# ShunyaoWang/quadruped_locomotion

Measured on AMD Instinct MI355X. Metric: control-step QP solves/sec (18-DoF, 4-contact) at 1/2/4/8 MI355X, higher is better.
Workload: dtype f64

## Files before the change

### quadruped_locomotion_amd/csrc/balance_coop.hpp

```cpp
#pragma once

#include "force_qp_coop.hpp"
#include "kernarg_mirror.hpp"
#include "qlamd.h"

namespace qlamd {
namespace coop {

struct CoopPtrs {
  const double *q, *pos, *quat, *linvel, *angvel, *dpos, *dquat, *dlinvel, *dangvel;
  const uint8_t *stance;
  const double *normals;
  const double *wrench;
  const uint8_t *live;
  int support_only;
  int32_t *iterations;
  const uint32_t *prev_working_set;
  uint32_t *working_set;
  uint32_t *warm_retries;
  int record_doubles;
  uint32_t *set_memory;
};

__host__ __device__ constexpr unsigned slot_legs_of(unsigned m) {
  unsigned perm = 0, k = 0;
  for (unsigned l = 0; l < 4; l++)
    if ((m >> l) & 1u) perm |= l << (2 * k++);
  for (unsigned l = 0; l < 4; l++)
    if (!((m >> l) & 1u)) perm |= l << (2 * k++);
  return perm;
}
__host__ __device__ constexpr unsigned long long slot_legs_table(int half) {
  unsigned long long t = 0;
  for (int m = 0; m < 8; m++) t |= (unsigned long long)slot_legs_of(8 * half + m) << (8 * m);
  return t;
}
__device__ __forceinline__ unsigned slot_legs(unsigned m) {
  constexpr unsigned long long lo = slot_legs_table(0), hi = slot_legs_table(1);
  return (unsigned)(((m & 8u) ? hi : lo) >> (8 * (m & 7u))) & 0xFFu;
}
template <int kKinds, class mask_t>
__device__ __forceinline__ mask_t working_set_to_slots(mask_t by_leg, unsigned perm) {
  constexpr mask_t rows = ((mask_t)1 << kKinds) - 1;
  mask_t out = 0;
#pragma unroll
  for (int sl = 0; sl < 4; sl++) out |= ((by_leg >> (kKinds * ((perm >> (2 * sl)) & 3u))) & rows) << (kKinds * sl);
  return out;
}
template <int kKinds, class mask_t>
__device__ __forceinline__ mask_t working_set_to_legs(mask_t by_slot, unsigned perm) {
  constexpr mask_t rows = ((mask_t)1 << kKinds) - 1;
  mask_t out = 0;
#pragma unroll
  for (int sl = 0; sl < 4; sl++) out |= ((by_slot >> (kKinds * sl)) & rows) << (kKinds * ((perm >> (2 * sl)) & 3u));
  return out;
}
__device__ __forceinline__ double from_leg_lane(double v, int aleg) {
  const int addr = (((int)threadIdx.x & 48) | (4 * aleg) | ((int)threadIdx.x & 3)) << 2;
  return __hiloint2double(__builtin_amdgcn_ds_bpermute(addr, __double2hiint(v)),
                          __builtin_amdgcn_ds_bpermute(addr, __double2loint(v)));
}

constexpr int kCoopNrmDoubles = 12 * 64;

template <bool kPerLeg, int kBlock = 64, bool kWarm = false, bool kParkInputs = false, bool kThroughput = false, bool kSmallForm = true,
          bool kTable = false>
__device__ __forceinline__ bool coop_robot(const DeviceParams &P, const CoopPtrs &s, int64_t irobot, bool robot_live_in,
                                           double *lds_tab, double *lds_row, double *lds_nrm,
                                           double *__restrict__ tau_out,
                                           double *__restrict__ grf_out, int32_t *__restrict__ status_out, bool cold = false) {
  bool robot_live = robot_live_in;
  const int lr = threadIdx.x & 15;
  const int leg = lr >> 2, c = lr & 3;
  const bool comp = c < 3;
  const int myidx = 3 * leg + c;
  const double eps = 2.220446049250313e-16;
  const double inf = INFINITY;

  QL_STAMP(0);
  constexpr int kTabLoads = (4 * kTabPerLeg + kBlock - 1) / kBlock;
  double tabv[kTabLoads];
#pragma unroll
  for (int j = 0; j < kTabLoads; j++) {
    const int idx = (int)threadIdx.x + kBlock * j;
    tabv[j] = P.legtab[idx < 4 * kTabPerLeg ? idx : 4 * kTabPerLeg - 1];
  }
  const int64_t i_in = irobot;
  const int64_t kS12 = s.record_doubles ? s.record_doubles : 12, kS4 = s.record_doubles ? s.record_doubles : 4,
                kS3 = s.record_doubles ? s.record_doubles : 3, kSB = 4;
  double quat[4], dquat[4], pos[3], linvel[3], angvel[3], dpos[3], dlinvel[3], dangvel[3];
  {
    const double2 *a2 = reinterpret_cast<const double2 *>(s.quat + kS4 * i_in);
    const double2 *b2 = reinterpret_cast<const double2 *>(s.dquat + kS4 * i_in);
    double2 v = a2[0]; quat[0] = v.x; quat[1] = v.y;
    v = a2[1]; quat[2] = v.x; quat[3] = v.y;
    v = b2[0]; dquat[0] = v.x; dquat[1] = v.y;
    v = b2[1]; dquat[2] = v.x; dquat[3] = v.y;
#pragma unroll
    for (int k = 0; k < 3; k++) {
      pos[k] = s.pos[kS3 * i_in + k]; linvel[k] = s.linvel[kS3 * i_in + k]; angvel[k] = s.angvel[kS3 * i_in + k];
      dpos[k] = s.dpos[kS3 * i_in + k]; dlinvel[k] = s.dlinvel[kS3 * i_in + k]; dangvel[k] = s.dangvel[kS3 * i_in + k];
    }
  }
  const uint32_t sm = *reinterpret_cast<const uint32_t *>(s.stance + kSB * i_in);
  double qj = s.q[kS12 * i_in + (comp ? myidx : 0)];
  const uint8_t alive = s.live ? s.live[i_in] : (uint8_t)1;
  unsigned warm_set = 0u;
  bool build_set = false;
  static_assert(!kTable || kWarm, "the table is a warm start");
  uint4 mem = make_uint4(0u, 0u, 0u, 0u);
  if constexpr (kTable) mem = reinterpret_cast<const uint4 *>(s.set_memory)[i_in];
  else if constexpr (kWarm) warm_set = (s.prev_working_set && !cold) ? s.prev_working_set[i_in] : 0u;
  double wr[6] = {0.0, 0.0, 0.0, 0.0, 0.0, 0.0};
  if (s.wrench) {
#pragma unroll
    for (int k = 0; k < 6; k++) wr[k] = s.wrench[6 * i_in + k];
  }
  double nWl[3] = {0.0, 0.0, 1.0};
  if (kPerLeg) { nWl[0] = s.normals[12 * i_in + 3 * leg]; nWl[1] = s.normals[12 * i_in + 3 * leg + 1]; nWl[2] = s.normals[12 * i_in + 3 * leg + 2]; }
  robot_live = robot_live && alive != 0;
  const unsigned stance = robot_live ? (((sm & 0xFFu) ? 1u : 0u) | ((sm & 0xFF00u) ? 2u : 0u) |
                                        ((sm & 0xFF0000u) ? 4u : 0u) | ((sm & 0xFF000000u) ? 8u : 0u))
                                     : 0u;
  const int nS = __popc(stance);
  if constexpr (kTable) {
    const unsigned slot = QLAMD_SET_MEMORY_SLOT(stance);
    warm_set = slot == 0u ? mem.x : slot == 1u ? mem.y : slot == 2u ? mem.z : mem.w;
  }
  if constexpr (kWarm) {
    const unsigned from = (warm_set >> 20) & 0xFu;
    warm_set = (from != 0u && from != stance) ? 0u : (warm_set & 0xFFFFFu);
    if constexpr (kTable) build_set = from != stance;
    else build_set = s.prev_working_set != nullptr && !cold && from != stance;
  }
  const unsigned perm = slot_legs(stance);
  const int aleg = (int)((perm >> (2 * leg)) & 3u);
  reinterpret_cast<int2 *>(lds_nrm + 64 * 11)[(int)threadIdx.x & 63] = make_int2((int)i_in, (3 * aleg + c) | ((int)perm << 8) | ((int)stance << 16));
  const bool on = leg < nS;
  const unsigned stance_slots = (1u << nS) - 1u;
  const bool permuted = __builtin_amdgcn_ballot_w64(perm != 0xE4u) != 0ull;
  if (permuted) {
    qj = from_leg_lane(qj, aleg);
    if (kPerLeg) { nWl[0] = from_leg_lane(nWl[0], aleg); nWl[1] = from_leg_lane(nWl[1], aleg); nWl[2] = from_leg_lane(nWl[2], aleg); }
  }
#pragma unroll
  for (int j = 0; j < kTabLoads; j++) {
    const int idx = (int)threadIdx.x + kBlock * j;
    if (idx < 4 * kTabPerLeg) lds_tab[idx] = tabv[j];
  }
  __syncthreads();

  QL_STAMP(1); QL_QP_BLOCK_STAMP(4);
  double Rm[9], gB[3], b[6];
  double wr_d[3] = {0.0, 0.0, 0.0}, wr_dw = 1.0, wr_k = 2.0;
  bool wr_slow = false;
  quat_to_matrix(quat, Rm);
  {
    const double gW[3] = {0.0, 0.0, -P.grav};
    irot(Rm, gW, gB);
    RobotIn in;
#pragma unroll
    for (int k = 0; k < 3; k++) {
      in.pos[k] = pos[k]; in.linvel[k] = linvel[k]; in.angvel[k] = angvel[k];
      in.dpos[k] = dpos[k]; in.dlinvel[k] = dlinvel[k]; in.dangvel[k] = dangvel[k];
    }
#pragma unroll
    for (int k = 0; k < 4; k++) { in.quat[k] = quat[k]; in.dquat[k] = dquat[k]; }
    in.has_wrench = false;
    wr_dw = 0.0;
    {
      const double *qd = in.dquat, *qm = in.quat;
      const double aw = qd[0], ax = -qd[1], ay = -qd[2], az = -qd[3];
      wr_dw = aw * qm[0] - ax * qm[1] - ay * qm[2] - az * qm[3];
      wr_d[0] = aw * qm[1] + ax * qm[0] + ay * qm[3] - az * qm[2];
      wr_d[1] = aw * qm[2] - ax * qm[3] + ay * qm[0] + az * qm[1];
      wr_d[2] = aw * qm[3] + ax * qm[2] - ay * qm[1] + az * qm[0];
      const double s2r = 1.0 - wr_dw * wr_dw;
      const double s2 = vmin(vmax(s2r, 0.0), 0.01);
      double p = 34459425.0 / 3530096640.0;
      p = fma(p, s2, 2027025.0 / 175472640.0);
      p = fma(p, s2, 135135.0 / 9676800.0);
      p = fma(p, s2, 10395.0 / 599040.0);
      p = fma(p, s2, 945.0 / 42240.0);
      p = fma(p, s2, 105.0 / 3456.0);
      p = fma(p, s2, 15.0 / 336.0);
      p = fma(p, s2, 3.0 / 40.0);
      p = fma(p, s2, 1.0 / 6.0);
      p = fma(p, s2, 1.0);
      wr_k = 2.0 * p;
      wr_slow = !(s2r < 0.01) || !(wr_dw > 0.0);
    }
    {
      double e_p[3], e_v[3], e_w[3];
#pragma unroll
      for (int k = 0; k < 3; k++) {
        e_p[k] = in.dpos[k] - in.pos[k];
        e_v[k] = in.dlinvel[k] - in.linvel[k];
        e_w[k] = in.dangvel[k] - in.angvel[k];
      }
      const double ff[3] = {in.dlinvel[0], in.dlinvel[1], 0.0};
      const double gfb[3] = {0.0, 0.0, P.kp_t[2] * e_p[2]};
      const double gdb[3] = {0.0, 0.0, P.kd_t[2] * e_v[2]};
// ... 47 lines not shown
    for (int a = 0; a < 3; a++) Rn[a] = Rc[0] * Rs[a] + Rc[1] * Rs[3 + a] + Rc[2] * Rs[6 + a];
    Rc[0] = Rn[0]; Rc[1] = Rn[1]; Rc[2] = Rn[2];
    Hk[k] = m * pc + (Rn[0] * mcom[0] + Rn[1] * mcom[1] + Rn[2] * mcom[2]);
    if (k < 3) { zax[k] = Rn[2]; pj[k] = pc; }
  }
  const double foot = (comp && on) ? pc : 0.0;
  const auto qcross = [&](double a, double bq) -> double {
    const double a1 = dpp<0xC9>(a), a2 = dpp<0xD2>(a);
    const double b1 = dpp<0xC9>(bq), b2 = dpp<0xD2>(bq);
    return a1 * b2 - a2 * b1;
  };
  double Jrow[3], Gq[3];
  {
    const double my_g = pick3(gB, c);
    double Hs = Hk[3];
    double M = tab[kTabMass + 3];
#pragma unroll
    for (int k = 2; k >= 0; k--) {
      Hs += Hk[k];
      M += tab[kTabMass + k];
      const double d = pc - pj[k];
      const double jc = qcross(zax[k], d);
      Jrow[k] = sel(comp, jc, 0.0);
      const double h = Hs - M * pj[k];
      const double zh = qcross(zax[k], h);
      Gq[k] = -quad_sum(sel(comp, my_g * zh, 0.0));
    }
  }

  if (__builtin_amdgcn_ballot_w64(wr_slow) != 0ull) {
    const double s2 = 1.0 - wr_dw * wr_dw;
    double k = 2.0;
    if (s2 >= 1e-12) k = 2.0 * acos(wr_dw) / sqrt(s2);
    const double dk = wr_slow ? k - wr_k : 0.0;
#pragma unroll
    for (int a = 0; a < 3; a++) b[3 + a] -= P.kp_r[a] * dk * wr_d[a];
  }
  if (s.wrench) {
#pragma unroll
    for (int k = 0; k < 6; k++) b[k] = wr[k];
  }
#pragma unroll
  for (int k = 0; k < 3; k++) {
    lds_nrm[64 * (5 + k) + ((int)threadIdx.x & 63)] = Jrow[k];
    lds_nrm[64 * (8 + k) + ((int)threadIdx.x & 63)] = Gq[k];
  }
  asm volatile("" ::: "memory");
  static_assert(!kParkInputs || kBlock == 64, "the parked inputs take the model table's place: one wavefront per workgroup");
  if constexpr (kParkInputs) {
    lds_tab[(int)threadIdx.x & 63] = foot;
#pragma unroll
    for (int k = 0; k < 6; k++) lds_tab[64 + 6 * (((int)threadIdx.x & 63) >> 4) + k] = b[k];
  }

  QL_STAMP(3); QL_QP_BLOCK_STAMP(5);
  double myn = 0.0, myt1 = 0.0, myt2 = 0.0;
  double nb[3], t1[3], t2[3];
  {
    const double ey[3] = {0.0, 1.0, 0.0}, ez[3] = {0.0, 0.0, 1.0};
    double yB[3], nW[3];
    irot(Rm, ey, yB);
    if (kPerLeg) { nW[0] = nWl[0]; nW[1] = nWl[1]; nW[2] = nWl[2]; }
    else rot(Rm, ez, nW);
    irot(Rm, nW, nb);
    cross3(nb, yB, t1);
    double nn = rsqrt_nr(dot3(t1, t1));
    t1[0] *= nn; t1[1] *= nn; t1[2] *= nn;
    cross3(nb, t1, t2);
    nn = rsqrt_nr(dot3(t2, t2));
    t2[0] *= nn; t2[1] *= nn; t2[2] *= nn;
    myn = pick3(nb, c); myt1 = pick3(t1, c); myt2 = pick3(t2, c);
  }
  const double mu = P.mu, f_min = P.f_min;

  QL_STAMP(4);
  QL_STAMP(5);
  double x;
  int qp_iters;
  unsigned long long final_set = 0ull;
  const bool two_legs = __builtin_amdgcn_ballot_w64(nS > 2) == 0ull;
  int status = kStatusOk;
  const auto solve = [&](auto Legs) {
    ForceQp Q;
    if constexpr (kParkInputs) {
      asm volatile("" ::: "memory");
      const double foot_l = lds_tab[(int)threadIdx.x & 63];
      double b_l[6];
#pragma unroll
      for (int k = 0; k < 6; k++) b_l[k] = lds_tab[64 + 6 * (((int)threadIdx.x & 63) >> 4) + k];
      force_qp_objective(P.S, P.w_reg, foot_l, stance_slots, comp && on, b_l, nullptr, 0.0, Q.Gm, Q.g0);
    } else {
      force_qp_objective(P.S, P.w_reg, foot, stance_slots, comp && on, b, nullptr, 0.0, Q.Gm, Q.g0);
    }
#pragma unroll
    for (int k = 0; k < 3; k++) { Q.nb[k] = nb[k]; Q.t1[k] = t1[k]; Q.t2[k] = t2[k]; }
    Q.myn = myn; Q.myt1 = myt1; Q.myt2 = myt2;
    Q.mu = mu; Q.f_min = f_min;
    Q.on = on; Q.comp = comp; Q.nS = nS; Q.refine_passes = P.refine_passes;
    Q.warm = 0ull; Q.stance = stance_slots;
    Q.build_set = build_set;
    if constexpr (kWarm) Q.warm = permuted ? working_set_to_slots<5, unsigned>(warm_set, perm) : warm_set;
    status = force_qp_coop<false, kWarm, decltype(Legs)::value, !kThroughput>(Q, lds_row, lds_nrm, x, qp_iters, &final_set);
  };
  if constexpr (kSmallForm) {
    int small_form = __builtin_amdgcn_readfirstlane(two_legs ? 1 : 0);
    asm volatile("" : "+s"(small_form));
    if (small_form != 0) solve(std::integral_constant<int, 2>{});
    int large_form = __builtin_amdgcn_readfirstlane(1 - small_form);
    asm volatile("" : "+s"(large_form));
    if (large_form != 0) solve(std::integral_constant<int, 4>{});
  } else {
    (void)two_legs;
    solve(std::integral_constant<int, 4>{});
  }
  const int2 parked = reinterpret_cast<const int2 *>(lds_nrm + 64 * 11)[(int)threadIdx.x & 63];
  const int64_t i = parked.x;
  const int aidx = parked.y & 15;
  if constexpr (kWarm) {
    if (permuted) final_set = working_set_to_legs<5, unsigned>((unsigned)final_set, ((unsigned)parked.y >> 8) & 0xFFu);
  }
  if (status == kStatusNotPd) {
    if (lr == 0 && robot_live) {
      status_out[i] = kStatusNotPd;
      if (s.iterations) s.iterations[i] = 0;
      if constexpr (kWarm) { if (s.working_set) s.working_set[i] = 0u; }
      if constexpr (kTable) s.set_memory[4 * i + QLAMD_SET_MEMORY_SLOT((unsigned)parked.y >> 16)] = 0u;
    }
    if (comp && robot_live && !P.keep_on_failure && (on || !s.support_only)) { tau_out[12 * i + aidx] = 0.0; if (grf_out) grf_out[12 * i + aidx] = 0.0; }
    return false;
  }

  QL_STAMP(8);
  {
    const bool live = on && status == kStatusOk;
    const double fx = live ? -x : 0.0;
    double Jr[3], Gr[3];
#pragma unroll
    for (int k = 0; k < 3; k++) {
      Jr[k] = lds_nrm[64 * (5 + k) + ((int)threadIdx.x & 63)];
      Gr[k] = lds_nrm[64 * (8 + k) + ((int)threadIdx.x & 63)];
    }
    const double t0 = quad_sum(sel(comp, Jr[0] * fx, 0.0)) + Gr[0];
    const double t1 = quad_sum(sel(comp, Jr[1] * fx, 0.0)) + Gr[1];
    const double t2 = quad_sum(sel(comp, Jr[2] * fx, 0.0)) + Gr[2];
    double t = sel(c == 0, t0, sel(c == 1, t1, t2));
    t = t > P.tau_max ? P.tau_max : t;
    t = t < -P.tau_max ? -P.tau_max : t;
    if (comp && robot_live && !(P.keep_on_failure && status != kStatusOk) && (on || !s.support_only)) {
      tau_out[12 * i + aidx] = live ? t : 0.0;
      if (grf_out) grf_out[12 * i + aidx] = live ? x : 0.0;
    }
    if (lr == 0 && robot_live) {
      status_out[i] = status;
      if (s.iterations) s.iterations[i] = qp_iters;
      if constexpr (kWarm) {
        const uint32_t word = status == kStatusOk ? ((uint32_t)final_set | (((uint32_t)parked.y >> 16 & 0xFu) << 20)) : 0u;
        if (s.working_set) s.working_set[i] = word;
        if constexpr (kTable)
          s.set_memory[4 * i + QLAMD_SET_MEMORY_SLOT((unsigned)parked.y >> 16)] = (P.warm_fallback == 2 && final_set != 0ull) ? 0u : word;
      }
    }
  }
  QL_STAMP(9);
  QL_STAMP(10);
  const bool rejected = kWarm && robot_live && (status == kStatusWarmRejected || (P.warm_fallback == 2 && status == kStatusOk && final_set != 0ull));
  if constexpr (kWarm) {
    if (rejected && lr == 0 && s.warm_retries) atomicAdd(s.warm_retries, 1u);
  }
  return rejected;
}

template <class Args>
__device__ __forceinline__ const Args *kernel_arguments_again() {
  typedef __attribute__((address_space(4))) const char kernarg_char;
  kernarg_char *kp = (kernarg_char *)__builtin_amdgcn_kernarg_segment_ptr();
  asm volatile("" : "+s"(kp));
  return (const Args *)kp;
}

}
}
```

### quadruped_locomotion_amd/csrc/balance_core.hpp

```cpp
#pragma once

#include <math.h>
#include <stdint.h>

#if defined(__HIPCC__)
#define QL_HD __host__ __device__ __forceinline__
#define QL_UNROLL _Pragma("unroll")
#define QL_NOUNROLL _Pragma("nounroll")
#define QL_HD_CALL __host__ __device__ __attribute__((noinline))
#else
#define QL_HD inline
#define QL_UNROLL
#define QL_NOUNROLL
#define QL_HD_CALL inline
#endif

namespace qlamd {

constexpr int kStatusOk = 0, kStatusInfeasible = 1, kStatusNotPd = 2, kStatusMaxIter = 3, kStatusDependentEquality = 5;
constexpr int kMaxOuter = 200;

struct DeviceParams {
  double kp_t[3], kd_t[3], kff_t[3];
  double kp_r[3], kd_r[3], kff_r[3];
  double S[6];
  double w_reg, mu, f_min, tau_max;
  double grav;
  double Fg_scale;
  double Tg_arm[3];
  double legtab[4 * 88];
  int refine_passes;
  int keep_on_failure;
  int warm_fallback;
};
constexpr int kTabR0 = 0, kTabXyz = 36, kTabMass = 48, kTabMcom = 52, kTabInertia = 64, kTabPerLeg = 88;

struct RobotIn {
  double q[12];
  double pos[3], quat[4], linvel[3], angvel[3];
  double dpos[3], dquat[4], dlinvel[3], dangvel[3];
  unsigned stance;
  bool has_wrench;
  double wrench[6];
};

#if defined(__HIP_DEVICE_COMPILE__)
QL_HD double ql_rcp(double x) {
  double y = __builtin_amdgcn_rcp(x);
  y = y + y * (1.0 - x * y);
  y = y + y * (1.0 - x * y);
  return y;
}
QL_HD double ql_rsqrt(double x) {
  double y = __builtin_amdgcn_rsq(x);
  y = y + y * (0.5 - 0.5 * x * y * y);
  y = y + y * (0.5 - 0.5 * x * y * y);
  return y;
}
#else
QL_HD double ql_rcp(double x) { return 1.0 / x; }
QL_HD double ql_rsqrt(double x) { return 1.0 / sqrt(x); }
#endif


QL_HD void cross3(const double a[3], const double b[3], double c[3]) {
  c[0] = a[1] * b[2] - a[2] * b[1];
  c[1] = a[2] * b[0] - a[0] * b[2];
  c[2] = a[0] * b[1] - a[1] * b[0];
}
QL_HD double dot3(const double a[3], const double b[3]) { return a[0] * b[0] + a[1] * b[1] + a[2] * b[2]; }

QL_HD void sincos_pio4(double x, double &s, double &c) {
  const double z = x * x;
  const double S1 = -1.66666666666666324348e-01, S2 = 8.33333333332248946124e-03,
               S3 = -1.98412698298579493134e-04, S4 = 2.75573137070700676789e-06,
               S5 = -2.50507602534068634195e-08, S6 = 1.58969099521155010221e-10;
  const double C1 = 4.16666666666666019037e-02, C2 = -1.38888888888741095749e-03,
               C3 = 2.48015872894767294178e-05, C4 = -2.75573143513906633035e-07,
               C5 = 2.08757232129817482790e-09, C6 = -1.13596475577881948265e-11;
  const double ps = S1 + z * (S2 + z * (S3 + z * (S4 + z * (S5 + z * S6))));
  s = x + x * z * ps;
  const double pc = z * (C1 + z * (C2 + z * (C3 + z * (C4 + z * (C5 + z * C6)))));
  c = 1.0 - (0.5 * z - z * pc);
}
QL_HD void sincos_reduced(double x, double &s, double &c) {
  const double two_over_pi = 6.36619772367581382433e-01;
  const double pio2_hi = 1.57079632673412561417e+00;
  const double pio2_lo = 6.07710050650619224932e-11;
  const double kf = rint(x * two_over_pi);
  const int k = (int)kf;
  const double r = (x - kf * pio2_hi) - kf * pio2_lo;
  double sr, cr;
  sincos_pio4(r, sr, cr);
  const bool swap = (k & 1) != 0;
  const double s0 = swap ? cr : sr, c0 = swap ? sr : cr;
  s = (k & 2) ? -s0 : s0;
  c = ((k + 1) & 2) ? -c0 : c0;
}

QL_HD void quat_to_matrix(const double q[4], double R[9]) {
  const double w = q[0], x = q[1], y = q[2], z = q[3];
  const double tx = 2.0 * x, ty = 2.0 * y, tz = 2.0 * z;
  const double twx = tx * w, twy = ty * w, twz = tz * w;
  const double txx = tx * x, txy = ty * x, txz = tz * x;
  const double tyy = ty * y, tyz = tz * y, tzz = tz * z;
  R[0] = 1.0 - (tyy + tzz); R[1] = txy - twz;         R[2] = txz + twy;
  R[3] = txy + twz;         R[4] = 1.0 - (txx + tzz); R[5] = tyz - twx;
  R[6] = txz - twy;         R[7] = tyz + twx;         R[8] = 1.0 - (txx + tyy);
}
QL_HD void rot(const double R[9], const double v[3], double o[3]) {
  QL_UNROLL for (int i = 0; i < 3; i++) o[i] = R[i * 3] * v[0] + R[i * 3 + 1] * v[1] + R[i * 3 + 2] * v[2];
}
QL_HD void irot(const double R[9], const double v[3], double o[3]) {
// ... 605 lines not shown
```

### quadruped_locomotion_amd/csrc/force_qp_coop.hpp

```cpp
#pragma once

#include "coop_lanes.hpp"

#if defined(__FAST_MATH__) || (defined(__FINITE_MATH_ONLY__) && __FINITE_MATH_ONLY__)
#error "force_qp_coop.hpp needs IEEE inf / NaN semantics: do not build this translation unit with -ffast-math / -ffinite-math-only"
#endif

#ifndef QL_QP_BLOCK_STAMP
#define QL_QP_BLOCK_STAMP(slot) QL_BLOCK_STAMP(slot)
#endif
namespace qlamd {
namespace coop {

constexpr int kCoopLdsDoubles = 12 * 12;
constexpr int kMaxRefinePasses = 8;
#ifndef QLAMD_REFINE_AGAIN
#define QLAMD_REFINE_AGAIN 1e-3
#endif
constexpr double kRefineAgain = QLAMD_REFINE_AGAIN;
constexpr int kDropSlot = 48, kZeroSlot = 60, kWarmSlot = 61;
constexpr int kForceQpNrmRows = 5, kForceQpNrmRowsTorque = 8;
template <class T>
constexpr T one_v = T(1);
constexpr int kStatusWarmRejected = 6;
struct ForceQp {
  double Gm[12];
  double g0;
  double nb[3], t1[3], t2[3];
  double myn, myt1, myt2;
  double mu, f_min;
  bool on, comp;
  int nS;
  int refine_passes;
  double jrow[3], jcol[3];
  double tq_up, tq_lo;
  unsigned long long warm;
  unsigned stance;
  bool build_set;
};

__device__ __forceinline__ void force_qp_objective(const double S[6], double w_reg, double foot, unsigned stance, bool row_on,
                                                   const double F[6], const double *jrow, double w_tau_jt0, double Gm[12],
                                                   double &g0, double w_tau = 0.0) {
  const int lr = threadIdx.x & 15, leg = lr >> 2, c = lr & 3;
  const int myidx = 3 * leg + c;
  double r[4][3];
  static_for<12>([&](auto J) { constexpr int j = J; r[j / 3][j % 3] = bcv<j>(foot); });
  const double rl[3] = {quad_bc<0>(foot), quad_bc<1>(foot), quad_bc<2>(foot)};
  const double a[3] = {sel(c == 1, -rl[2], sel(c == 2, rl[1], 0.0)), sel(c == 0, rl[2], sel(c == 2, -rl[0], 0.0)),
                       sel(c == 0, -rl[1], sel(c == 1, rl[0], 0.0))};
  const double sa[3] = {S[3] * a[0], S[4] * a[1], S[5] * a[2]};
  const double Sfc = pick3(S, c);
#pragma unroll
  for (int m = 0; m < 4; m++) {
    const bool both = row_on && ((stance >> m) & 1u);
    const double xp = r[m][0], yp = r[m][1], zp = r[m][2];
    const double e0 = sa[1] * zp - sa[2] * yp;
    const double e1 = -sa[0] * zp + sa[2] * xp;
    const double e2 = sa[0] * yp - sa[1] * xp;
    Gm[3 * m + 0] = both ? e0 + (c == 0 ? Sfc : 0.0) : 0.0;
    Gm[3 * m + 1] = both ? e1 + (c == 1 ? Sfc : 0.0) : 0.0;
    Gm[3 * m + 2] = both ? e2 + (c == 2 ? Sfc : 0.0) : 0.0;
  }
  if (jrow) {
    double jj[3];
    static_for<3>([&](auto Bq) {
      constexpr int bq = Bq;
      jj[bq] = jrow[0] * quad_bc<bq>(jrow[0]) + jrow[1] * quad_bc<bq>(jrow[1]) + jrow[2] * quad_bc<bq>(jrow[2]);
    });
#pragma unroll
    for (int m = 0; m < 4; m++) {
      const bool own = row_on && m == leg;
#pragma unroll
      for (int bq = 0; bq < 3; bq++) Gm[3 * m + bq] += own ? w_tau * jj[bq] : 0.0;
    }
  }
#pragma unroll
  for (int j = 0; j < 12; j++)
    if (c < 3 && j == myidx) Gm[j] += row_on ? w_reg : 1.0;
  const double Fc = pick3(F, c);
  const double ST[3] = {S[3] * F[3], S[4] * F[4], S[5] * F[5]};
  const double g0v = -(Sfc * Fc + (a[0] * ST[0] + a[1] * ST[1] + a[2] * ST[2]) + w_tau_jt0);
  g0 = sel(row_on, g0v, 0.0);
}

template <bool kTorque, bool kWarm = false, int kLegs = 4, bool kRounds = true>
__device__ __forceinline__ int force_qp_coop(const ForceQp &Q, double *lds_row, double *lds_nrm, double &x, int &iters_out,
                                             unsigned long long *ws_out = nullptr) {
  using mask_t = std::conditional_t<kTorque, unsigned long long, unsigned>;
  constexpr int kKinds = kTorque ? 11 : 5;
  static_assert(kLegs == 2 || kLegs == 4, "legs in front of the row");
  constexpr int kV = 3 * kLegs;
  const int lr = threadIdx.x & 15, leg = lr >> 2, c = lr & 3;
  const bool comp = Q.comp && leg < kLegs, on = Q.on, row_on = comp && on;
  const int myidx = 3 * leg + c, nS = Q.nS;
  const double eps = 2.220446049250313e-16;
  const double inf = INFINITY;
  const double mu = Q.mu, f_min = Q.f_min, g0 = Q.g0;
  const double myn = Q.myn, myt1 = Q.myt1, myt2 = Q.myt2;
  const double *nb = Q.nb, *t1 = Q.t1, *t2 = Q.t2, *Gm = Q.Gm;
  double H[kV];
  double c1 = 0.0, c2 = 0.0;
  {
#pragma unroll
    for (int j = 0; j < kV; j++) H[j] = Gm[j];
    {
      double diag = 0.0;
#pragma unroll
      for (int j = 0; j < kV; j++) diag = (j == myidx) ? Gm[j] : diag;
      c1 = row_sum(sel(row_on, diag, 0.0));
    }
    bool bad = false;
    double my_pivot = 1.0;
    double d = bcv<0>(H[0]);
    static_for<kV>([&](auto K) {
      constexpr int k = K;
      bad = bad || !(d > 0.0);
      const double p = rcp_nr1(d);
      const bool piv = comp && (myidx == k);
      my_pivot = piv ? d : my_pivot;
      const double f = piv ? (1.0 - p) : H[k] * p;
      const double nf = -f;
      if constexpr (k < kV - 1) {
        fmac_bc<lane_of(k), true>(H[k + 1], H[k + 1], nf);
        d = bcv<k + 1>(H[k + 1]);
      }
      static_for<kV>([&](auto J) {
        constexpr int j = J;
        if constexpr (j != k && j != k + 1) fmac_bc<lane_of(k), (k == kV - 1 && j == 0)>(H[j], H[j], nf);
      });
      H[k] = piv ? p : nf;
    });
    const double rp = rsqrt_nr(my_pivot);
    c2 = row_sum(sel(row_on, rp, 0.0));
    if (bad && nS > 0) { iters_out = 0; return kStatusNotPd; }
  }

  QL_STAMP(5);
  x = 0.0;
  {
    const double ng0 = -g0;
    double xa[3] = {0.0, 0.0, 0.0};
    static_for<kV>([&](auto J) { constexpr int j = J; fmac_bc<lane_of(j), j == 0>(xa[j % 3], ng0, H[j]); });
    x = (xa[0] + xa[1]) + xa[2];
  }

  QL_STAMP(6); QL_QP_BLOCK_STAMP(6);
  double Ns[kV];
#pragma unroll
  for (int j = 0; j < kV; j++) Ns[j] = 0.0;
  double u = 0.0;
  int idk = 0;
  unsigned used = 0;
  int q = 0, iters = 0, status = kStatusOk;
  mask_t act_mask = 0, excl = 0;
  const double psi_tol = (double)(kKinds * nS) * eps * c1 * c2 * 100.0;
  double rnorm2 = 1.0;
  unsigned long long done_m = 0ull;
  int ip = 0;
  double sp = 0.0, ucand = 0.0, npj = 0.0;
  const double fa = c == 0 ? 1.0 : c == 1 ? -1.0 : 0.0, fb = c == 2 ? 1.0 : c == 3 ? -1.0 : 0.0;
  const double Wf0 = mu * nb[0] + (fa * t1[0] + fb * t2[0]), Wf1 = mu * nb[1] + (fa * t1[1] + fb * t2[1]),
               Wf2 = mu * nb[2] + (fa * t1[2] + fb * t2[2]);
  const mask_t one = 1;
  const mask_t maskf = on ? (one << (kKinds * leg + c + 1)) : 0, maskm = (on && c == 0) ? (one << (kKinds * leg)) : 0;
  const mask_t masku = (kTorque && on && comp) ? (one << (kKinds * leg + 5 + 2 * c)) : 0, maskl = masku << 1;
  constexpr int kTagBits = kTorque ? 2 : 1;
  constexpr unsigned kTagMask = (1u << (4 + kTagBits)) - 1u;
  const unsigned tagf = (unsigned)lr << kTagBits, tagm = tagf | 1u;
  const int row_addr = ((int)threadIdx.x & 48) << 2;
  const unsigned lanebit = 1u << lr;
  {
    const double nrm[5] = {myn, mu * myn + myt1, mu * myn - myt1, mu * myn + myt2, mu * myn - myt2};
#pragma unroll
    for (int k = 0; k < 5; k++) lds_nrm[64 * k + ((int)threadIdx.x & 63)] = nrm[k];
    lds_row[kZeroSlot] = 0.0;
    if constexpr (kTorque) {
#pragma unroll
      for (int k = 0; k < 3; k++) lds_nrm[64 * (5 + k) + ((int)threadIdx.x & 63)] = Q.jrow[k];
    }
  }
  const int nt_slot = comp ? kDropSlot + myidx : kZeroSlot;
  double zb = 0.0;
  double s_up = 0.0, s_lo = 0.0;
  const auto slacks = [&](double xx, double &s_min, double &s_fric) {
    const double x0 = quad_bc<0>(xx), x1 = quad_bc<1>(xx), x2 = quad_bc<2>(xx);
    s_fric = fma(Wf2, x2, fma(Wf1, x1, Wf0 * x0));
    s_min = fma(nb[2], x2, fma(nb[1], x1, fma(nb[0], x0, -f_min)));
    if constexpr (kTorque) {
      const double d = fma(Q.jcol[2], x2, fma(Q.jcol[1], x1, Q.jcol[0] * x0));
      s_up = Q.tq_up + d;
      s_lo = Q.tq_lo - d;
    }
  };
  const auto violation = [&](double s_min, double s_fric) -> double {
    double v = vmin(0.0, s_fric) + sel(c == 0, vmin(0.0, s_min), 0.0);
    if constexpr (kTorque) v += sel(comp, vmin(0.0, s_up) + vmin(0.0, s_lo), 0.0);
    return v;
  };
  const auto umax_dpp = [](unsigned k, auto Ctrl) -> unsigned {
    constexpr int ctrl = decltype(Ctrl)::value;
    const unsigned o = (unsigned)__builtin_amdgcn_mov_dpp((int)k, ctrl, 0xF, 0xF, true);
    return k > o ? k : o;
  };

  const auto latch = [&](bool newly) {
    if (newly) {
      lds_row[lr] = x;
      reinterpret_cast<int2 *>(lds_row + 16)[lr] = make_int2((int)used, idk);
      reinterpret_cast<int2 *>(lds_row + 32)[lr] = make_int2(q | (iters << 8), status);
      lds_row[nt_slot] = 0.0;
      lds_nrm[64 * 1 + ((int)threadIdx.x & 63)] = 0.0;
      zb = 0.0625; npj = 0.0;
    }
  };
  double vec = 0.0, hc = 0.0, nc = 0.0;
  const auto update_and_select = [&](auto Mode, bool resel, bool fresh, bool finished = false) -> bool {
    constexpr int kMode = decltype(Mode)::value;
    constexpr bool kUpd = kMode != 0;
    if constexpr (kMode == 1) {
      iters += (resel && fresh) ? 1 : 0;
      excl = (resel && fresh) ? 0 : excl;
    } else {
// ... 550 lines not shown
```

### quadruped_locomotion_amd/csrc/params_build.hpp

```cpp
#pragma once

#include <math.h>
#include <stdlib.h>
#include <string.h>

#include "balance_core.hpp"
#include "qlamd.h"
#include "qlamd_robot_constants.h"

namespace qlamd {

inline void default_balance_params(qlamd_balance_params *p) {
  const double kp_t[3] = {5000, 5000, 10000}, kd_t[3] = {5000, 4000, 5000}, kff_t[3] = {10, 10, 100};
  const double kp_r[3] = {10000, 10000, 4000}, kd_r[3] = {1000, 1000, 1000}, kff_r[3] = {0.2, 0.2, 1000};
  const double S[6] = {1, 5, 1, 10, 10, 5};
  const double hips[4][3] = {{0.42, 0.075, 0.0}, {0.42, -0.075, 0.0}, {-0.42, -0.075, 0.0}, {-0.42, 0.075, 0.0}};
  memcpy(p->kp_trans, kp_t, sizeof(kp_t)); memcpy(p->kd_trans, kd_t, sizeof(kd_t));
  memcpy(p->kff_trans, kff_t, sizeof(kff_t));
  memcpy(p->kp_rot, kp_r, sizeof(kp_r)); memcpy(p->kd_rot, kd_r, sizeof(kd_r));
  memcpy(p->kff_rot, kff_r, sizeof(kff_r));
  memcpy(p->force_weights, S, sizeof(S));
  p->regularizer = 0.0001; p->friction = 0.6; p->min_normal_force = 10.0;
  p->torque_limit = 300.0;
  p->torso_mass = 27.0;
  for (int i = 0; i < 4; i++) p->leg_mass[i] = 6.0;
  p->gravity = 9.8;
  p->grav_comp_percentage = 1.0;
  p->com_in_base[0] = p->com_in_base[1] = p->com_in_base[2] = 0.0;
  memcpy(p->hip_in_base, hips, sizeof(hips));
}

inline void default_robot_model(qlamd_robot_model *m) {
  memcpy(m->joint_xyz, QLAMD_JOINT_XYZ, sizeof(m->joint_xyz));
  memcpy(m->joint_rpy, QLAMD_JOINT_RPY, sizeof(m->joint_rpy));
  memcpy(m->link_mass, QLAMD_LINK_MASS, sizeof(m->link_mass));
  memcpy(m->link_com, QLAMD_LINK_COM, sizeof(m->link_com));
  memcpy(m->link_inertia, QLAMD_LINK_INERTIA, sizeof(m->link_inertia));
  m->base_mass = QLAMD_BASE_MASS;
  memcpy(m->base_com, QLAMD_BASE_COM, sizeof(m->base_com));
  memcpy(m->base_inertia, QLAMD_BASE_INERTIA, sizeof(m->base_inertia));
}

inline void rpy_to_matrix(const double rpy[3], double R[9]) {
  const double cr = cos(rpy[0]), sr = sin(rpy[0]);
  const double cp = cos(rpy[1]), sp = sin(rpy[1]);
  const double cy = cos(rpy[2]), sy = sin(rpy[2]);
  R[0] = cy * cp; R[1] = cy * sp * sr - sy * cr; R[2] = cy * sp * cr + sy * sr;
  R[3] = sy * cp; R[4] = sy * sp * sr + cy * cr; R[5] = sy * sp * cr - cy * sr;
  R[6] = -sp;     R[7] = cp * sr;                R[8] = cp * cr;
}

inline void build_device_params(const qlamd_balance_params &p, const qlamd_robot_model &m, DeviceParams *d) {
  memset(d, 0, sizeof(*d));
  for (int i = 0; i < 3; i++) {
    d->kp_t[i] = p.kp_trans[i]; d->kd_t[i] = p.kd_trans[i]; d->kff_t[i] = p.kff_trans[i];
    d->kp_r[i] = p.kp_rot[i];   d->kd_r[i] = p.kd_rot[i];   d->kff_r[i] = p.kff_rot[i];
  }
  for (int i = 0; i < 6; i++) d->S[i] = p.force_weights[i];
  d->w_reg = p.regularizer; d->mu = p.friction; d->f_min = p.min_normal_force; d->tau_max = p.torque_limit;
  d->grav = p.gravity;
  d->refine_passes = 1;
  d->keep_on_failure = 0;
  d->warm_fallback = 1;
  double mass = p.torso_mass;
  double arm[3] = {p.torso_mass * p.com_in_base[0], p.torso_mass * p.com_in_base[1], p.torso_mass * p.com_in_base[2]};
  for (int l = 0; l < 4; l++) {
    mass += p.leg_mass[l];
    for (int i = 0; i < 3; i++) arm[i] += p.leg_mass[l] * (p.hip_in_base[l][i] - p.com_in_base[i]);
  }
  d->Fg_scale = p.grav_comp_percentage * mass;
  for (int i = 0; i < 3; i++) d->Tg_arm[i] = p.grav_comp_percentage * arm[i];
  for (int l = 0; l < 4; l++) {
    double *tab = d->legtab + kTabPerLeg * l;
    for (int k = 0; k < 4; k++) {
      rpy_to_matrix(m.joint_rpy[l][k], tab + kTabR0 + 9 * k);
      tab[kTabMass + k] = m.link_mass[l][k];
      for (int i = 0; i < 3; i++) {
        tab[kTabXyz + 3 * k + i] = m.joint_xyz[l][k][i];
        tab[kTabMcom + 3 * k + i] = m.link_mass[l][k] * m.link_com[l][k][i];
      }
      for (int i = 0; i < 6; i++) tab[kTabInertia + 6 * k + i] = m.link_inertia[l][k][i];
    }
  }
}

}
```

### quadruped_locomotion_amd/csrc/balance_coop_body.hpp

```cpp
  double *tab = lds, *rows = lds + 4 * kTabPerLeg, *nrm = rows + 4 * kCoopWaves * coop::kCoopLdsDoubles;
  const DeviceParams &P = *Pp;
  const int row = threadIdx.x >> 4, wave = threadIdx.x >> 6;
  unsigned block = blockIdx.x;
  QL_BLOCK_STAMP(0);
  if constexpr (kPlaced) {
    if (s.shadow_blocks) {
      if (block < (unsigned)s.shadow_blocks) {
        placement_wave(s.prev_iterations, B, s.place_throughput, s.next_order, (lds_u32 *)lds, block, (uint32_t)s.shadow_blocks,
                       (uint32_t)s.shadow_chunk, s.place_throughput ? reinterpret_cast<const uint32_t *>(s.stance) : nullptr, s.place_hist, s.place_sync,
                       s.place_wait);
        return;
      }
      block -= (unsigned)s.shadow_blocks;
      __builtin_amdgcn_s_setprio(3);
    }
  }
  int64_t i = (int64_t)block * (4 * kCoopWaves) + row;
  bool live = i < B;
  if (!live) i = B - 1;
  if constexpr (kPlaced) {
    if constexpr (kMinWaves == 2) {
      if (s.shadow_blocks == 0 && s.next_order && live && (threadIdx.x & 15) == 0) s.next_order[i] = (int32_t)i;
    }
    if (s.order) {
      const int64_t o = s.order[i];
      live = live && o >= 0 && o < B;
      i = live ? o : B - 1;
    }
  }
  const coop::CoopPtrs cp{s.q, s.pos, s.quat, s.linvel, s.angvel, s.dpos, s.dquat, s.dlinvel, s.dangvel, s.stance,
                          s.normals, s.wrench, s.live, s.support_only, kPlaced ? s.iterations : nullptr,
                          kWarm ? s.prev_working_set : nullptr, kWarm ? s.working_set : nullptr, kWarm ? s.warm_retries : nullptr,
                          s.record_doubles, kTable ? s.set_memory : nullptr};
#ifdef QLAMD_STAMPS
#pragma unroll 1
  for (int rep = 0; rep < 2; rep++)
#endif
  {
    const bool rejected = coop::coop_robot<kPerLeg, 64 * kCoopWaves, kWarm, kMinWaves == 3 && !kWarm && kPlaced, kMinWaves == 3, kPlaced, kTable>(
        P, cp, i, live, tab, rows + row * coop::kCoopLdsDoubles, nrm + wave * coop::kCoopNrmDoubles, tau, grf, status);
    QL_BLOCK_STAMP(3);
    if constexpr (kWarm) {
      if (__builtin_expect(P.warm_fallback && __builtin_amdgcn_ballot_w64(rejected) != 0ull, 0)) {
        __syncthreads();
        if constexpr (kTable) balance_table_retry<kPerLeg, kMinWaves>(coop::kernel_arguments_again<BalanceCoopArgs>(), lds, rejected);
        else balance_cold_retry<kPerLeg, kMinWaves>(coop::kernel_arguments_again<BalanceCoopArgs>(), lds, rejected);
      }
    }
  }
```

Baseline: 299.9 million.

## Replace Gauss-Jordan Hessian inverse with closed-form structured inverse for 4-leg force QP

Adds a closed-form inverse of the force-QP Hessian that exploits its structure: diagonal regularizer plus low-rank wrench terms, reduced to a 3x3 Schur complement per row. It is used for the non-torque, 4-leg case and falls back to the cooperative Gauss-Jordan elimination when any lane detects ill-conditioning. The goal is to remove the serial cross-lane elimination cost. In exchange it adds precomputed sqrt and inverse parameters, extra fields in the QP struct, and possible numerical differences compared with the elimination path.

```diff
diff --git a/quadruped_locomotion_amd/csrc/balance_coop.hpp b/quadruped_locomotion_amd/csrc/balance_coop.hpp
--- a/quadruped_locomotion_amd/csrc/balance_coop.hpp
+++ b/quadruped_locomotion_amd/csrc/balance_coop.hpp
@@ -331,15 +331,17 @@
   int status = kStatusOk;
   const auto solve = [&](auto Legs) {
     ForceQp Q;
+    double b_l[6];
     if constexpr (kParkInputs) {
       asm volatile("" ::: "memory");
       const double foot_l = lds_tab[(int)threadIdx.x & 63];
-      double b_l[6];
 #pragma unroll
       for (int k = 0; k < 6; k++) b_l[k] = lds_tab[64 + 6 * (((int)threadIdx.x & 63) >> 4) + k];
-      force_qp_objective(P.S, P.w_reg, foot_l, stance_slots, comp && on, b_l, nullptr, 0.0, Q.Gm, Q.g0);
+      force_qp_objective(P.S, P.w_reg, foot_l, stance_slots, comp && on, b_l, nullptr, 0.0, Q.Gm, Q.g0, 0.0, &Q.foot);
+      Q.F = b_l;
     } else {
-      force_qp_objective(P.S, P.w_reg, foot, stance_slots, comp && on, b, nullptr, 0.0, Q.Gm, Q.g0);
+      force_qp_objective(P.S, P.w_reg, foot, stance_slots, comp && on, b, nullptr, 0.0, Q.Gm, Q.g0, 0.0, &Q.foot);
+      Q.F = b;
     }
 #pragma unroll
     for (int k = 0; k < 3; k++) { Q.nb[k] = nb[k]; Q.t1[k] = t1[k]; Q.t2[k] = t2[k]; }
@@ -348,6 +350,7 @@
     Q.on = on; Q.comp = comp; Q.nS = nS; Q.refine_passes = P.refine_passes;
     Q.warm = 0ull; Q.stance = stance_slots;
     Q.build_set = build_set;
+    Q.inv = StructuredInverseParams{P.S, P.S_sqrt, P.w_reg, P.w_reg_inv, P.w_reg_rsqrt};
     if constexpr (kWarm) Q.warm = permuted ? working_set_to_slots<5, unsigned>(warm_set, perm) : warm_set;
     status = force_qp_coop<false, kWarm, decltype(Legs)::value, !kThroughput>(Q, lds_row, lds_nrm, x, qp_iters, &final_set);
   };
diff --git a/quadruped_locomotion_amd/csrc/balance_core.hpp b/quadruped_locomotion_amd/csrc/balance_core.hpp
--- a/quadruped_locomotion_amd/csrc/balance_core.hpp
+++ b/quadruped_locomotion_amd/csrc/balance_core.hpp
@@ -29,6 +29,8 @@
   double Fg_scale;
   double Tg_arm[3];
   double legtab[4 * 88];
+  double S_sqrt[6];
+  double w_reg_inv, w_reg_rsqrt;
   int refine_passes;
   int keep_on_failure;
   int warm_fallback;
diff --git a/quadruped_locomotion_amd/csrc/force_qp_coop.hpp b/quadruped_locomotion_amd/csrc/force_qp_coop.hpp
--- a/quadruped_locomotion_amd/csrc/force_qp_coop.hpp
+++ b/quadruped_locomotion_amd/csrc/force_qp_coop.hpp
@@ -1,6 +1,7 @@
 #pragma once
 
 #include "coop_lanes.hpp"
+#include "force_qp_inverse.hpp"
 
 #if defined(__FAST_MATH__) || (defined(__FINITE_MATH_ONLY__) && __FINITE_MATH_ONLY__)
 #error "force_qp_coop.hpp needs IEEE inf / NaN semantics: do not build this translation unit with -ffast-math / -ffinite-math-only"
@@ -36,14 +37,19 @@
   double tq_up, tq_lo;
   unsigned long long warm;
   unsigned stance;
+  double foot;
+  const double *F;
+  StructuredInverseParams inv;
   bool build_set;
 };
 
 __device__ __forceinline__ void force_qp_objective(const double S[6], double w_reg, double foot, unsigned stance, bool row_on,
                                                    const double F[6], const double *jrow, double w_tau_jt0, double Gm[12],
-                                                   double &g0, double w_tau = 0.0) {
+                                                   double &g0, double w_tau = 0.0, double *foot_on = nullptr) {
   const int lr = threadIdx.x & 15, leg = lr >> 2, c = lr & 3;
   const int myidx = 3 * leg + c;
+  foot = sel(row_on, foot, 0.0);
+  if (foot_on) *foot_on = foot;
   double r[4][3];
   static_for<12>([&](auto J) { constexpr int j = J; r[j / 3][j % 3] = bcv<j>(foot); });
   const double rl[3] = {quad_bc<0>(foot), quad_bc<1>(foot), quad_bc<2>(foot)};
@@ -101,7 +107,23 @@
   const double *nb = Q.nb, *t1 = Q.t1, *t2 = Q.t2, *Gm = Q.Gm;
   double H[kV];
   double c1 = 0.0, c2 = 0.0;
-  {
+#ifdef QLAMD_NO_STRUCTURED_INVERSE
+  constexpr bool kStructured = false;
+#else
+  constexpr bool kStructured = !kTorque && kLegs == 4;
+#endif
+  bool gauss_jordan = !kStructured;
+  x = 0.0;
+  if constexpr (kStructured) {
+    double r[4][3];
+    static_for<12>([&](auto J) { constexpr int j = J; r[j / 3][j % 3] = bcv<j>(Q.foot); });
+    const double rl[3] = {quad_bc<0>(Q.foot), quad_bc<1>(Q.foot), quad_bc<2>(Q.foot)};
+    bool ill;
+    const bool bad = structured_inverse_row<4>(Q.inv, r, rl, Q.stance, nS, leg, c, comp, row_on, Q.F, H, c1, c2, x, ill);
+    if (bad && nS > 0) { iters_out = 0; return kStatusNotPd; }
+    gauss_jordan = __builtin_amdgcn_ballot_w64(ill && nS > 0) != 0ull;
+  }
+  if (gauss_jordan) {
 #pragma unroll
     for (int j = 0; j < kV; j++) H[j] = Gm[j];
     {
@@ -137,8 +159,7 @@
   }
 
   QL_STAMP(5);
-  x = 0.0;
-  {
+  if (gauss_jordan) {
     const double ng0 = -g0;
     double xa[3] = {0.0, 0.0, 0.0};
     static_for<kV>([&](auto J) { constexpr int j = J; fmac_bc<lane_of(j), j == 0>(xa[j % 3], ng0, H[j]); });
diff --git a/quadruped_locomotion_amd/csrc/force_qp_inverse.hpp b/quadruped_locomotion_amd/csrc/force_qp_inverse.hpp
--- /dev/null
+++ b/quadruped_locomotion_amd/csrc/force_qp_inverse.hpp
@@ -0,0 +1,77 @@
+#pragma once
+
+#include "balance_core.hpp"
+
+namespace qlamd {
+
+struct StructuredInverseParams {
+  const double *S, *S_sqrt;
+  double w, w_inv, w_rsqrt;
+};
+
+QL_HD double si_sel(bool p, double a, double b) { return p ? a : b; }
+template <int kLegs>
+QL_HD bool structured_inverse_row(const StructuredInverseParams &P, const double (*r)[3], const double rl[3], unsigned stance, int n,
+                                  int leg, int c, bool comp, bool row_on, const double F[6], double *H, double &c1, double &c2, double &x0,
+                                  bool &ill) {
+  const double *S = P.S, *s = P.S_sqrt;
+  const double w = P.w, g = P.w_inv, nd = (double)n;
+  double R[3] = {0.0, 0.0, 0.0}, Wxx = 0.0, Wyy = 0.0, Wzz = 0.0, Wxy = 0.0, Wxz = 0.0, Wyz = 0.0;
+  QL_UNROLL
+  for (int m = 0; m < kLegs; m++) {
+    R[0] += r[m][0]; R[1] += r[m][1]; R[2] += r[m][2];
+    Wxx = fma(r[m][0], r[m][0], Wxx); Wyy = fma(r[m][1], r[m][1], Wyy); Wzz = fma(r[m][2], r[m][2], Wzz);
+    Wxy = fma(r[m][0], r[m][1], Wxy); Wxz = fma(r[m][0], r[m][2], Wxz); Wyz = fma(r[m][1], r[m][2], Wyz);
+  }
+  c1 = fma(nd, fma(3.0, w, (S[0] + S[1]) + S[2]), fma(S[3], Wyy + Wzz, fma(S[4], Wxx + Wzz, S[5] * (Wxx + Wyy))));
+  c2 = 3.0 * nd * P.w_rsqrt;
+  const double D[3] = {fma(nd, S[0], w), fma(nd, S[1], w), fma(nd, S[2], w)};
+  const double k[3] = {S[0] * ql_rcp(D[0]), S[1] * ql_rcp(D[1]), S[2] * ql_rcp(D[2])};
+  const double R00 = R[0] * R[0], R11 = R[1] * R[1], R22 = R[2] * R[2];
+  const double Q00 = (Wyy + Wzz) - fma(k[1], R22, k[2] * R11), Q11 = (Wxx + Wzz) - fma(k[0], R22, k[2] * R00),
+               Q22 = (Wxx + Wyy) - fma(k[0], R11, k[1] * R00);
+  const double Q01 = fma(k[2] * R[0], R[1], -Wxy), Q02 = fma(k[1] * R[0], R[2], -Wxz), Q12 = fma(k[0] * R[1], R[2], -Wyz);
+  const double E00 = fma(S[3], Q00, w), E11 = fma(S[4], Q11, w), E22 = fma(S[5], Q22, w);
+  const double E01 = (s[3] * s[4]) * Q01, E02 = (s[3] * s[5]) * Q02, E12 = (s[4] * s[5]) * Q12;
+  const double a00 = fma(E11, E22, -(E12 * E12)), a01 = fma(E02, E12, -(E01 * E22)), a02 = fma(E01, E12, -(E02 * E11));
+  const double a11 = fma(E00, E22, -(E02 * E02)), a12 = fma(E01, E02, -(E00 * E12)), a22 = fma(E00, E11, -(E01 * E01));
+  const double det = fma(E00, a00, fma(E01, a01, E02 * a02));
+  const bool bad = !(w > 0.0) || !(E00 > 0.0) || !(a22 > 0.0) || !(det > 0.0);
+  {
+    const double trW = (Wxx + Wyy) + Wzz;
+    ill = !(4096.0 * det >= (fma(S[3], trW, w) * fma(S[4], trW, w)) * fma(S[5], trW, w));
+  }
+  const double di = ql_rcp(det);
+  const double Z00 = a00 * di, Z01 = a01 * di, Z02 = a02 * di, Z11 = a11 * di, Z12 = a12 * di, Z22 = a22 * di;
+  const double kc = si_sel(c == 0, k[0], si_sel(c == 1, k[1], si_sel(c == 2, k[2], 0.0)));
+  const double rt[3] = {fma(-kc, R[0], rl[0]), fma(-kc, R[1], rl[1]), fma(-kc, R[2], rl[2])};
+  const double on = si_sel(row_on, 1.0, 0.0);
+  const double b0 = (on * s[3]) * si_sel(c == 1, -rt[2], si_sel(c == 2, rt[1], 0.0));
+  const double b1 = (on * s[4]) * si_sel(c == 0, rt[2], si_sel(c == 2, -rt[0], 0.0));
+  const double b2 = (on * s[5]) * si_sel(c == 0, -rt[1], si_sel(c == 1, rt[0], 0.0));
+  const double v0 = s[3] * fma(Z00, b0, fma(Z01, b1, Z02 * b2)), v1 = s[4] * fma(Z01, b0, fma(Z11, b1, Z12 * b2)),
+               v2 = s[5] * fma(Z02, b0, fma(Z12, b1, Z22 * b2));
+  const double q0 = fma(v1, R[2], -(v2 * R[1])), q1 = fma(v2, R[0], -(v0 * R[2])), q2 = fma(v0, R[1], -(v1 * R[0]));
+  {
+    const double y0 = k[0] * (si_sel(c == 0, on, 0.0) - q0), y1 = k[1] * (si_sel(c == 1, on, 0.0) - q1),
+                 y2 = k[2] * (si_sel(c == 2, on, 0.0) - q2);
+    x0 = fma(y0, F[0], fma(y1, F[1], fma(y2, F[2], fma(v0, F[3], fma(v1, F[4], v2 * F[5])))));
+  }
+  const double dg = si_sel(comp, si_sel(row_on, g, 1.0), 0.0);
+  const double t0 = (k[0] * g) * (q0 - si_sel(c == 0, on, 0.0)), t1 = (k[1] * g) * (q1 - si_sel(c == 1, on, 0.0)),
+               t2 = (k[2] * g) * (q2 - si_sel(c == 2, on, 0.0));
+  const double d0 = t0 + si_sel(c == 0, dg, 0.0), d1 = t1 + si_sel(c == 1, dg, 0.0), d2 = t2 + si_sel(c == 2, dg, 0.0);
+  const double u0 = -g * v0, u1 = -g * v1, u2 = -g * v2;
+  QL_UNROLL
+  for (int m = 0; m < kLegs; m++) {
+    const bool own = m == leg, col = ((stance >> m) & 1u) != 0u;
+    const double e0 = si_sel(own, d0, si_sel(col, t0, 0.0)), e1 = si_sel(own, d1, si_sel(col, t1, 0.0)),
+                 e2 = si_sel(own, d2, si_sel(col, t2, 0.0));
+    H[3 * m + 0] = fma(u1, r[m][2], fma(-u2, r[m][1], e0));
+    H[3 * m + 1] = fma(u2, r[m][0], fma(-u0, r[m][2], e1));
+    H[3 * m + 2] = fma(u0, r[m][1], fma(-u1, r[m][0], e2));
+  }
+  return bad;
+}
+
+}
diff --git a/quadruped_locomotion_amd/csrc/params_build.hpp b/quadruped_locomotion_amd/csrc/params_build.hpp
--- a/quadruped_locomotion_amd/csrc/params_build.hpp
+++ b/quadruped_locomotion_amd/csrc/params_build.hpp
@@ -58,6 +58,9 @@
   }
   for (int i = 0; i < 6; i++) d->S[i] = p.force_weights[i];
   d->w_reg = p.regularizer; d->mu = p.friction; d->f_min = p.min_normal_force; d->tau_max = p.torque_limit;
+  for (int i = 0; i < 6; i++) d->S_sqrt[i] = sqrt(p.force_weights[i]);
+  d->w_reg_inv = p.regularizer > 0.0 ? 1.0 / p.regularizer : 0.0;
+  d->w_reg_rsqrt = p.regularizer > 0.0 ? 1.0 / sqrt(p.regularizer) : 0.0;
   d->grav = p.gravity;
   d->refine_passes = 1;
   d->keep_on_failure = 0;
```

After: 300.7 million (median of 2 runs). Within noise of the previous version (+0.3%).

## Speculate robot order and restructure input loads for latency-bound kernel head

Applied to the files above, without the earlier changes.

In the two-wave configuration, the order lookup moves into the robot solver. When the order is known to be the identity (no shadow placement), the input loads are issued speculatively at the unpermuted index and reissued only if any lane's order word differs. Otherwise the loads wait on the order word. Conditional loads are made branchless by aliasing a valid pointer, and kernel-argument values are pinned in scalar registers with empty asm statements. The aim is to shorten the dependent-load chain at kernel start, at the cost of occasional duplicate loads and higher register pressure.

```diff
diff --git a/quadruped_locomotion_amd/csrc/balance_coop.hpp b/quadruped_locomotion_amd/csrc/balance_coop.hpp
--- a/quadruped_locomotion_amd/csrc/balance_coop.hpp
+++ b/quadruped_locomotion_amd/csrc/balance_coop.hpp
@@ -61,14 +61,21 @@
                           __builtin_amdgcn_ds_bpermute(addr, __double2loint(v)));
 }
 
+struct SlotOrder {
+  const int32_t *order = nullptr;
+  int64_t batch = 0;
+  bool speculate = false;
+};
+
 constexpr int kCoopNrmDoubles = 12 * 64;
 
 template <bool kPerLeg, int kBlock = 64, bool kWarm = false, bool kParkInputs = false, bool kThroughput = false, bool kSmallForm = true,
-          bool kTable = false>
+          bool kTable = false, bool kLatencyHead = false>
 __device__ __forceinline__ bool coop_robot(const DeviceParams &P, const CoopPtrs &s, int64_t irobot, bool robot_live_in,
                                            double *lds_tab, double *lds_row, double *lds_nrm,
                                            double *__restrict__ tau_out,
-                                           double *__restrict__ grf_out, int32_t *__restrict__ status_out, bool cold = false) {
+                                           double *__restrict__ grf_out, int32_t *__restrict__ status_out, bool cold = false,
+                                           const SlotOrder ord = SlotOrder{}) {
   bool robot_live = robot_live_in;
   const int lr = threadIdx.x & 15;
   const int leg = lr >> 2, c = lr & 3;
@@ -78,6 +85,10 @@
   const double inf = INFINITY;
 
   QL_STAMP(0);
+  int32_t order_word = (int32_t)irobot;
+  if constexpr (kLatencyHead) {
+    if (ord.order != nullptr) order_word = ord.order[irobot];
+  }
   constexpr int kTabLoads = (4 * kTabPerLeg + kBlock - 1) / kBlock;
   double tabv[kTabLoads];
 #pragma unroll
@@ -85,39 +96,71 @@
     const int idx = (int)threadIdx.x + kBlock * j;
     tabv[j] = P.legtab[idx < 4 * kTabPerLeg ? idx : 4 * kTabPerLeg - 1];
   }
-  const int64_t i_in = irobot;
-  const int64_t kS12 = s.record_doubles ? s.record_doubles : 12, kS4 = s.record_doubles ? s.record_doubles : 4,
-                kS3 = s.record_doubles ? s.record_doubles : 3, kSB = 4;
+  int64_t i_in = irobot;
   double quat[4], dquat[4], pos[3], linvel[3], angvel[3], dpos[3], dlinvel[3], dangvel[3];
-  {
-    const double2 *a2 = reinterpret_cast<const double2 *>(s.quat + kS4 * i_in);
-    const double2 *b2 = reinterpret_cast<const double2 *>(s.dquat + kS4 * i_in);
-    double2 v = a2[0]; quat[0] = v.x; quat[1] = v.y;
-    v = a2[1]; quat[2] = v.x; quat[3] = v.y;
-    v = b2[0]; dquat[0] = v.x; dquat[1] = v.y;
-    v = b2[1]; dquat[2] = v.x; dquat[3] = v.y;
-#pragma unroll
-    for (int k = 0; k < 3; k++) {
-      pos[k] = s.pos[kS3 * i_in + k]; linvel[k] = s.linvel[kS3 * i_in + k]; angvel[k] = s.angvel[kS3 * i_in + k];
-      dpos[k] = s.dpos[kS3 * i_in + k]; dlinvel[k] = s.dlinvel[kS3 * i_in + k]; dangvel[k] = s.dangvel[kS3 * i_in + k];
-    }
-  }
-  const uint32_t sm = *reinterpret_cast<const uint32_t *>(s.stance + kSB * i_in);
-  double qj = s.q[kS12 * i_in + (comp ? myidx : 0)];
-  const uint8_t alive = s.live ? s.live[i_in] : (uint8_t)1;
+  uint32_t sm;
+  double qj;
+  uint8_t alive;
   unsigned warm_set = 0u;
   bool build_set = false;
   static_assert(!kTable || kWarm, "the table is a warm start");
   uint4 mem = make_uint4(0u, 0u, 0u, 0u);
-  if constexpr (kTable) mem = reinterpret_cast<const uint4 *>(s.set_memory)[i_in];
-  else if constexpr (kWarm) warm_set = (s.prev_working_set && !cold) ? s.prev_working_set[i_in] : 0u;
   double wr[6] = {0.0, 0.0, 0.0, 0.0, 0.0, 0.0};
-  if (s.wrench) {
-#pragma unroll
-    for (int k = 0; k < 6; k++) wr[k] = s.wrench[6 * i_in + k];
-  }
   double nWl[3] = {0.0, 0.0, 1.0};
-  if (kPerLeg) { nWl[0] = s.normals[12 * i_in + 3 * leg]; nWl[1] = s.normals[12 * i_in + 3 * leg + 1]; nWl[2] = s.normals[12 * i_in + 3 * leg + 2]; }
+  const auto issue = [&]() {
+    const int64_t kS12 = s.record_doubles ? s.record_doubles : 12, kS4 = s.record_doubles ? s.record_doubles : 4,
+                  kS3 = s.record_doubles ? s.record_doubles : 3, kSB = 4;
+    {
+      const double2 *a2 = reinterpret_cast<const double2 *>(s.quat + kS4 * i_in);
+      const double2 *b2 = reinterpret_cast<const double2 *>(s.dquat + kS4 * i_in);
+      double2 v = a2[0]; quat[0] = v.x; quat[1] = v.y;
+      v = a2[1]; quat[2] = v.x; quat[3] = v.y;
+      v = b2[0]; dquat[0] = v.x; dquat[1] = v.y;
+      v = b2[1]; dquat[2] = v.x; dquat[3] = v.y;
+#pragma unroll
+      for (int k = 0; k < 3; k++) {
+        pos[k] = s.pos[kS3 * i_in + k]; linvel[k] = s.linvel[kS3 * i_in + k]; angvel[k] = s.angvel[kS3 * i_in + k];
+        dpos[k] = s.dpos[kS3 * i_in + k]; dlinvel[k] = s.dlinvel[kS3 * i_in + k]; dangvel[k] = s.dangvel[kS3 * i_in + k];
+      }
+    }
+    sm = *reinterpret_cast<const uint32_t *>(s.stance + kSB * i_in);
+    qj = s.q[kS12 * i_in + (comp ? myidx : 0)];
+    if constexpr (kLatencyHead) {
+      const uint8_t a = (s.live ? s.live : s.stance)[i_in];
+      alive = s.live ? a : (uint8_t)1;
+    } else {
+      alive = s.live ? s.live[i_in] : (uint8_t)1;
+    }
+    if constexpr (kTable) mem = reinterpret_cast<const uint4 *>(s.set_memory)[i_in];
+    else if constexpr (kWarm && kLatencyHead) {
+      const bool given = s.prev_working_set && !cold;
+      const uint32_t w = (given ? s.prev_working_set : reinterpret_cast<const uint32_t *>(s.stance))[i_in];
+      warm_set = given ? w : 0u;
+    } else if constexpr (kWarm) warm_set = (s.prev_working_set && !cold) ? s.prev_working_set[i_in] : 0u;
+    if (s.wrench) {
+#pragma unroll
+      for (int k = 0; k < 6; k++) wr[k] = s.wrench[6 * i_in + k];
+    }
+    if (kPerLeg) { nWl[0] = s.normals[12 * i_in + 3 * leg]; nWl[1] = s.normals[12 * i_in + 3 * leg + 1]; nWl[2] = s.normals[12 * i_in + 3 * leg + 2]; }
+  };
+  if constexpr (kLatencyHead) {
+    const bool guess = ord.order != nullptr && ord.speculate;
+    const auto seat = [&](int64_t o) {
+      robot_live = robot_live && o >= 0 && o < ord.batch;
+      i_in = robot_live ? o : ord.batch - 1;
+    };
+    if (ord.order != nullptr && !guess) {
+      asm volatile("" : "+v"(order_word));
+      seat(order_word);
+    }
+    issue();
+    if (guess && __builtin_amdgcn_ballot_w64(order_word != irobot) != 0ull) {
+      seat(order_word);
+      issue();
+    }
+  } else {
+    issue();
+  }
   robot_live = robot_live && alive != 0;
   const unsigned stance = robot_live ? (((sm & 0xFFu) ? 1u : 0u) | ((sm & 0xFF00u) ? 2u : 0u) |
                                         ((sm & 0xFF0000u) ? 4u : 0u) | ((sm & 0xFF000000u) ? 8u : 0u))
diff --git a/quadruped_locomotion_amd/csrc/balance_coop_body.hpp b/quadruped_locomotion_amd/csrc/balance_coop_body.hpp
--- a/quadruped_locomotion_amd/csrc/balance_coop_body.hpp
+++ b/quadruped_locomotion_amd/csrc/balance_coop_body.hpp
@@ -3,6 +3,16 @@
   const int row = threadIdx.x >> 4, wave = threadIdx.x >> 6;
   unsigned block = blockIdx.x;
   QL_BLOCK_STAMP(0);
+  constexpr bool kLatencyHead = kMinWaves == 2;
+  if constexpr (kLatencyHead) {
+    asm volatile("" ::"s"(s.q), "s"(s.pos), "s"(s.quat), "s"(s.linvel), "s"(s.angvel), "s"(s.dpos), "s"(s.dquat), "s"(s.dlinvel), "s"(s.dangvel));
+    asm volatile("" ::"s"(Pp), "s"(s.stance), "s"(s.wrench), "s"(s.live), "s"(s.support_only), "s"(s.record_doubles), "s"(B), "s"(tau),
+                 "s"(grf), "s"(status));
+    if constexpr (kPerLeg) asm volatile("" ::"s"(s.normals));
+    if constexpr (kPlaced) asm volatile("" ::"s"(s.order), "s"(s.next_order), "s"(s.iterations), "s"(s.shadow_blocks));
+    if constexpr (kTable) asm volatile("" ::"s"(s.set_memory), "s"(s.warm_retries));
+    else if constexpr (kWarm) asm volatile("" ::"s"(s.prev_working_set), "s"(s.working_set), "s"(s.warm_retries));
+  }
   if constexpr (kPlaced) {
     if (s.shadow_blocks) {
       if (block < (unsigned)s.shadow_blocks) {
@@ -18,11 +28,13 @@
   int64_t i = (int64_t)block * (4 * kCoopWaves) + row;
   bool live = i < B;
   if (!live) i = B - 1;
+  coop::SlotOrder slots;
   if constexpr (kPlaced) {
     if constexpr (kMinWaves == 2) {
-      if (s.shadow_blocks == 0 && s.next_order && live && (threadIdx.x & 15) == 0) s.next_order[i] = (int32_t)i;
-    }
-    if (s.order) {
+      const bool none = s.shadow_blocks == 0 && s.next_order;
+      if (none && live && (threadIdx.x & 15) == 0) s.next_order[i] = (int32_t)i;
+      slots = coop::SlotOrder{s.order, B, none};
+    } else if (s.order) {
       const int64_t o = s.order[i];
       live = live && o >= 0 && o < B;
       i = live ? o : B - 1;
@@ -37,8 +49,9 @@
   for (int rep = 0; rep < 2; rep++)
 #endif
   {
-    const bool rejected = coop::coop_robot<kPerLeg, 64 * kCoopWaves, kWarm, kMinWaves == 3 && !kWarm && kPlaced, kMinWaves == 3, kPlaced, kTable>(
-        P, cp, i, live, tab, rows + row * coop::kCoopLdsDoubles, nrm + wave * coop::kCoopNrmDoubles, tau, grf, status);
+    const bool rejected = coop::coop_robot<kPerLeg, 64 * kCoopWaves, kWarm, kMinWaves == 3 && !kWarm && kPlaced, kMinWaves == 3, kPlaced, kTable,
+                                           kLatencyHead>(
+        P, cp, i, live, tab, rows + row * coop::kCoopLdsDoubles, nrm + wave * coop::kCoopNrmDoubles, tau, grf, status, false, slots);
     QL_BLOCK_STAMP(3);
     if constexpr (kWarm) {
       if (__builtin_expect(P.warm_fallback && __builtin_amdgcn_ballot_w64(rejected) != 0ull, 0)) {
```

Measured after the change: 299.6 million before, 292.5 million after. 2.4% lower.
